# NVIDIA/CUDALibrarySamples

Measured on AMD Instinct MI355X. Metric: contraction GFLOP/s, fp32 einsum abcd,dcbe->ae, higher is better.
Workload: dtype f32

## Files before the change

### cudalibrarysamples_amd/csrc/host/api.cpp

```cpp
#include <algorithm>
#include <cmath>
#include <cstdio>
#include <cstdlib>
#include <cstring>
#include <new>
#include <optional>
#include <sstream>

#include <hip/hip_runtime.h>

#include "internal.hpp"

using namespace ctamd;

static const cutensorComputeDescriptor kCompute[6] = {
    {0, CUTENSOR_COMPUTE_16F}, {1, CUTENSOR_COMPUTE_16BF}, {2, CUTENSOR_COMPUTE_TF32},
    {3, CUTENSOR_COMPUTE_3XTF32}, {4, CUTENSOR_COMPUTE_32F}, {5, CUTENSOR_COMPUTE_64F}};
extern "C" {
const cutensorComputeDescriptor_t CUTENSOR_COMPUTE_DESC_16F    = &kCompute[0];
const cutensorComputeDescriptor_t CUTENSOR_COMPUTE_DESC_16BF   = &kCompute[1];
const cutensorComputeDescriptor_t CUTENSOR_COMPUTE_DESC_TF32   = &kCompute[2];
const cutensorComputeDescriptor_t CUTENSOR_COMPUTE_DESC_3XTF32 = &kCompute[3];
const cutensorComputeDescriptor_t CUTENSOR_COMPUTE_DESC_32F    = &kCompute[4];
const cutensorComputeDescriptor_t CUTENSOR_COMPUTE_DESC_64F    = &kCompute[5];
// ... 1796 lines not shown
        if (h->prof.enabled.load(std::memory_order_relaxed) && hipEventCreate(&e0) == hipSuccess && hipEventCreate(&e1) == hipSuccess)
            (void)hipEventRecord(e0, stream);
    }
    void end() {
        if (!e0 || !e1) return;
        (void)hipEventRecord(e1, stream);
        std::lock_guard<std::mutex> g(handle->prof.mtx);
        handle->prof.events.emplace_back(e0, e1);
    }
};
static bool mode_table_on_device(const cutensorHandle_t handle, cutensorPlan& plan) {
    if (plan.wideDev) return true;
    std::lock_guard<std::mutex> g(handle->mtx);
    if (!plan.wideDev) plan.wideDev = upload_mode_table(plan.wideTab);
    return plan.wideDev != nullptr;
}
static hipError_t launch_mode_table(const cutensorPlan& plan, const GettParams& p, const CallScalars& s, hipStream_t stream) {
    WideParams w = plan.wide;
    w.modes = plan.wideDev.get();
    w.A = p.A; w.B = p.B; w.C = p.C; w.D = p.D;
    w.alpha = p.alpha; w.beta = p.beta; w.alpha64 = s.a; w.beta64 = s.b;
    w.alphaIm = s.aIm; w.betaIm = s.bIm;
    g_launchCounts[1].fetch_add(1, std::memory_order_relaxed);
    return launch_gett_wide(w, (int)plan.dtype, plan.accumulate64, stream);
}
static hipError_t launch_strip_plan(const ContractionChoice& c, const GettKernelInfo& ki, const GettKernelInfo& ks, const GettParams& p, hipStream_t stream) {
    const uint32_t mInt = c.mInt, nInt = c.nInt, Mt = p.gM.total, Nt = p.gN.total, Lt = p.gL.total;
    GettParams q = p;
    q.tilesM = mInt / (uint32_t)ki.bm; q.tilesN = nInt / (uint32_t)ki.bn;
    q.nBlocks = q.tilesM * q.tilesN * Lt;
    const hipError_t err = ki.launch(q, stream);
    GettParams s2 = p;
    s2.mOrg = mInt; s2.nOrg = 0;
    s2.tilesM = (Mt - mInt + (uint32_t)ks.bm - 1u) / (uint32_t)ks.bm; s2.tilesN = (Nt + (uint32_t)ks.bn - 1u) / (uint32_t)ks.bn;
    s2.mOrg2 = 0; s2.nOrg2 = nInt;
    s2.tilesM2 = (mInt + (uint32_t)ks.bm - 1u) / (uint32_t)ks.bm; s2.tilesN2 = (Nt - nInt + (uint32_t)ks.bn - 1u) / (uint32_t)ks.bn;
    if (s2.tilesM * s2.tilesN == 0u) {
        s2.mOrg = s2.mOrg2; s2.nOrg = s2.nOrg2; s2.tilesM = s2.tilesM2; s2.tilesN = s2.tilesN2;
        s2.tilesM2 = s2.tilesN2 = 0;
    }
    s2.nBlocks = (s2.tilesM * s2.tilesN + s2.tilesM2 * s2.tilesN2) * Lt;
    return (err == hipSuccess && s2.nBlocks > 0u) ? ks.launch(s2, stream) : err;
}
static hipError_t launch_tiled(const cutensorHandle_t handle, const cutensorPlan& plan, GettParams& p, const CallScalars& s, void* workspace, hipStream_t stream) {
    const ContractionChoice& c = plan.choice;
    int count = 0;
    const GettKernelInfo* tab = kernel_table(c.family, &count);
    g_launchCounts[2 + c.family].fetch_add(1, std::memory_order_relaxed);
    p.partial = (c.splitK > 1) ? static_cast<float*>(workspace) : nullptr;
    int launchKernel = c.kernel;
    if (c.family == 0) {
        static const int policy = [] { const char* e = CTAMD_HOOK_ENV("CUTENSOR_AMD_PARTIAL_STORE"); return e ? (e[0] == 'p' ? 1 : e[0] == 'n' ? 2 : e[0] == 's' ? 3 : 0) : 0; }();
        p.partialPolicy = policy;
        p.noFlatStart = CTAMD_HOOK_ENV_IS("CUTENSOR_AMD_FLAT_START", '0') ? 1 : 0;
        if (plan.fusedFold) {
            uint32_t slot;
            {
                std::lock_guard<std::mutex> g(handle->mtx);
                slot = handle->syncNext++ % cutensorHandle::kSyncSlots;
            }
            p.sync = handle->syncPool + (size_t)slot * 16;
        }
    } else if (c.family == 1) {
        static const bool persistentForced = CTAMD_HOOK_ENV("CUTENSOR_AMD_H16_WAVES") != nullptr && h16_waves_variant() == H16_W4P;
        if (tab[launchKernel].variant == H16_W4P && s.b != 0.0 && p.cStrideN[0] != 1 && !persistentForced)
            launchKernel = h16_entry(H16_W4X, launchKernel - H16_W4P);
        g_lastH16Kernel.store(launchKernel, std::memory_order_relaxed);
    }
    ProfiledLaunch prof(handle, stream);
    hipError_t err = (c.family == 1 && c.stripKernel >= 0 && c.stripKernel < count) ? launch_strip_plan(c, tab[launchKernel], tab[c.stripKernel], p, stream)
                                                                                    : tab[launchKernel].launch(p, stream);
    prof.end();
    if (err != hipSuccess || c.splitK <= 1 || (c.family == 0 && (plan.fusedFold || handle->skipFold.load(std::memory_order_relaxed)))) return err;
    SplitKReduceParams r = plan.skr;
    r.partial = static_cast<float*>(workspace);
    r.C = p.C; r.D = p.D; r.alpha = p.alpha; r.beta = p.beta;
    r.alpha64 = s.a; r.beta64 = s.b; r.alphaIm = s.aIm; r.betaIm = s.bIm; r.conjC = p.conjC;
    r.noFlatStart = p.noFlatStart;
    return launch_splitk_fold(c.family, tab[c.kernel], r, stream);
}

cutensorStatus_t cutensorContract(const cutensorHandle_t handle, const cutensorPlan_t plan, const void* alpha,
                                  const void* A, const void* B, const void* beta, const void* C, void* D,
                                  void* workspace, uint64_t workspaceSize, cudaStream_t stream) try {
    if (handle == nullptr) return CUTENSOR_STATUS_NOT_INITIALIZED;
    if (plan == nullptr || plan->kind != OpKind::Contraction) return CUTENSOR_STATUS_INVALID_VALUE;
    if (alpha == nullptr || beta == nullptr || A == nullptr || B == nullptr || D == nullptr) return CUTENSOR_STATUS_INVALID_VALUE;
    const CallScalars s{scalar_as_double(alpha, plan->scalarType), scalar_as_double(beta, plan->scalarType), scalar_imag(alpha, plan->scalarType),
                        scalar_imag(beta, plan->scalarType)};
    const bool betaZero = (s.b == 0.0 && s.bIm == 0.0);
    if (!betaZero && C == nullptr) return CUTENSOR_STATUS_INVALID_VALUE;
    if (misaligned(A, plan->alignA) || misaligned(B, plan->alignB) || misaligned(D, plan->alignD) ||
        (!betaZero && misaligned(C, plan->alignC)))
        return CUTENSOR_STATUS_INVALID_VALUE;
    if (plan->requiredWorkspace > 0 && (workspace == nullptr || workspaceSize < plan->requiredWorkspace))
        return CUTENSOR_STATUS_INSUFFICIENT_WORKSPACE;
    switch (plan->planKind) {
        case PlanKind::LoneReduce:
        case PlanKind::Repack: return run_two_step(handle, *plan, alpha, A, B, beta, C, D, workspace, workspaceSize, stream);
        case PlanKind::Peeled: return run_peeled(handle, *plan, alpha, A, B, beta, C, D, workspace, workspaceSize, stream);
        case PlanKind::ModeTable:
            if (!mode_table_on_device(handle, *plan)) return CUTENSOR_STATUS_ALLOC_FAILED;
            break;
        default: break;
    }
    GettParams p = plan->gett;
    p.A = plan->view.swapped ? B : A;
// ... 425 lines not shown
```

### cudalibrarysamples_amd/csrc/kernels/gett_f32_stream.hip

```cpp
#include <hip/hip_runtime.h>
#include <stdint.h>
#include <stdlib.h>

#include <atomic>

#include "params.h"
#include "launch.h"
#include "gett_common.h"

namespace ctamd {

constexpr int kStreamBK = 32;

typedef uint32_t u32x4 __attribute__((ext_vector_type(4)));
#if defined(__HIP_DEVICE_COMPILE__)
typedef __amdgpu_buffer_rsrc_t BufRsrc;
#else
typedef int BufRsrc;
#endif
__device__ __forceinline__ BufRsrc make_rsrc(const float* base, uint32_t records = 0xffffffffu) {
#if defined(__HIP_DEVICE_COMPILE__)
    return __builtin_amdgcn_make_buffer_rsrc(const_cast<float*>(base), 0, (int)records, 0x00020000);
#else
    (void)base; (void)records; return 0;
#endif
}
__device__ __forceinline__ void store_wt_16(f32x4 v, BufRsrc rsrc, uint32_t byteOff) {
#if defined(__HIP_DEVICE_COMPILE__)
    __builtin_amdgcn_raw_buffer_store_b128(__builtin_bit_cast(u32x4, v), rsrc, (int)byteOff, 0,  16);
#else
    (void)v; (void)rsrc; (void)byteOff;
#endif
}
template <int AUX>
__device__ __forceinline__ void store_policy_16(f32x4 v, BufRsrc rsrc, uint32_t byteOff) {
#if defined(__HIP_DEVICE_COMPILE__)
    __builtin_amdgcn_raw_buffer_store_b128(__builtin_bit_cast(u32x4, v), rsrc, (int)byteOff, 0, AUX);
#else
    (void)v; (void)rsrc; (void)byteOff;
#endif
}
template <int AUX = 0>
__device__ __forceinline__ void lds_dma_16(BufRsrc rsrc, uint32_t laneBytes, uint32_t tileBytes, float* dst) {
#if defined(__HIP_DEVICE_COMPILE__)
    __builtin_amdgcn_raw_ptr_buffer_load_lds(rsrc, (__attribute__((address_space(3))) void*)dst, 16, (int)laneBytes, (int)tileBytes, 0, AUX);
#else
    (void)rsrc; (void)laneBytes; (void)tileBytes; (void)dst;
#endif
}

template <int LAY, int ROWS>
struct StreamOperand {
    static_assert(ROWS % 32 == 0, "tile rows must be a multiple of 32");
    static constexpr int PIECES   = ROWS / 8;
    static constexpr int PER_WAVE = PIECES / 4;
    static constexpr int FLOATS   = ROWS * kStreamBK;
    static constexpr int UR       = ROWS / 4;

    uint32_t src[PER_WAVE];

    template <int SLOT_K>
    __device__ __forceinline__ void init(const ModeGroup& gFree, const ModeGroup& gK, uint32_t row0, int wave, int lane) {
        const int64_t strideK0 = gK.stride[SLOT_K][0];
#pragma unroll
        for (int i = 0; i < PER_WAVE; ++i) {
// ... 137 lines not shown
                offB = sgpr((uint32_t)group_offset<1>(gK, k) * 4u);
            }
        }
    }
    __device__ static __forceinline__ uint32_t flat_div(const StreamFlatParams& f, int i, uint32_t n) {
        return __umulhi(n, f.kMagic[i]) >> ((f.kShifts >> (8 * i)) & 0xffu);
    }
    __device__ static __forceinline__ void flat_high(const StreamFlatParams& f, uint32_t hi, uint32_t& a, uint32_t& b) {
        const uint32_t d3 = flat_div(f, 2, hi), d2 = hi - d3 * f.kExt[2];
        a = d2 * f.kStrideA[2] + d3 * f.kStrideA[3];
        b = d2 * f.kStrideB[2] + d3 * f.kStrideB[3];
    }
    __device__ __forceinline__ void init(const StreamFlatParams& f, uint32_t k0) {
        const uint32_t E0 = f.kExt[0];
        n0 = sgpr(E0 / kStreamBK);
        e1 = sgpr(f.kExt[1]);
        const uint32_t q0 = flat_div(f, 0, k0), d0 = k0 - q0 * E0;
        j0 = sgpr(d0 / kStreamBK);
        hi = sgpr((e1 < 2) ? q0 : flat_div(f, 1, q0));
        j1 = sgpr(q0 - hi * e1);
        uint32_t a, b;
        flat_high(f, hi, a, b);
        offA = sgpr(d0 * f.kStrideA[0] + j1 * f.kStrideA[1] + a);
        offB = sgpr(d0 * f.kStrideB[0] + j1 * f.kStrideB[1] + b);
        stepA = sgpr((uint32_t)kStreamBK * f.kStrideA[0]);
        stepB = sgpr((uint32_t)kStreamBK * f.kStrideB[0]);
        wrapA = sgpr(f.kStrideA[1] - (n0 - 1) * stepA);
        wrapB = sgpr(f.kStrideB[1] - (n0 - 1) * stepB);
    }
    __device__ __forceinline__ void advance(const StreamFlatParams& f) {
        const bool c0 = (j0 + 1 == n0);
        j0 = c0 ? 0u : j0 + 1;
        offA += c0 ? wrapA : stepA;
        offB += c0 ? wrapB : stepB;
        j1 += c0 ? 1u : 0u;
        if (j1 == e1) {
            j1 = 0;
            hi += 1;
            if (hi * e1 * f.kExt[0] < f.kTotal) {
                uint32_t a, b;
                flat_high(f, hi, a, b);
                offA = sgpr(a);
                offB = sgpr(b);
            }
        }
    }
};

template <int BM_, int BN_, int LA_, int LB_, int S_, int ABL_ = 0, bool RAG_ = false>
struct StreamCfg {
    static constexpr int BM = BM_, BN = BN_, LA = LA_, LB = LB_, S = S_;
    static constexpr bool RAG = RAG_;
    static constexpr int ABL = ABL_;
    static constexpr bool FLAT = ABL_ == 6 || ABL_ == 7;
    static constexpr bool NT = ABL_ == 5 || ABL_ == 7;
    static constexpr int TM = BM / 32, TN = BN / 32;
};

#define CTAMD_WAIT_VMCNT(n) asm volatile("s_waitcnt vmcnt(%0)" ::"n"(n) : "memory")

template <class Cfg>
__global__ void __launch_bounds__(512, 2) gett_f32_stream_kernel(const GettParams p) {
    constexpr int BM = Cfg::BM, BN = Cfg::BN, BK = kStreamBK, S = Cfg::S;
    constexpr int TM = Cfg::TM, TN = Cfg::TN;
    using OpA = StreamOperand<Cfg::LA, BM>;
    using OpB = StreamOperand<Cfg::LB, BN>;
    constexpr int STAGE = OpA::FLOATS + OpB::FLOATS;
    constexpr int LOADS = OpA::PER_WAVE + OpB::PER_WAVE;
    static_assert(S >= 3 && S <= 6 && S * STAGE * 4 <= 160 * 1024, "LDS ring must fit 160 KiB");
    static_assert(LOADS * (S - 1) <= 63, "vmcnt is a 6-bit counter");
    __shared__ __attribute__((aligned(16))) float lds[S * STAGE];
    prefetch_kernarg<(int)sizeof(GettParams)>();

    const int tid  = threadIdx.x;
    const int lane = tid & 63;
    const int wave8 = __builtin_amdgcn_readfirstlane(tid >> 6);
    const int wave = wave8 & 3;
    const bool loader = wave8 >= 4;
    unsigned long long* tlog = p.timing ? p.timing + (size_t)blockIdx.x * 16 : nullptr;
    auto lane_now = []() -> int {
#if defined(__HIP_DEVICE_COMPILE__)
        return (int)__builtin_amdgcn_mbcnt_hi(~0u, __builtin_amdgcn_mbcnt_lo(~0u, 0u));
#else
        return 0;
#endif
    };
    auto stamp = [&](int slot) {
        if (tlog != nullptr && wave8 == 0 && lane_now() == 0) tlog[slot] = (slot >= 5 && slot != 7) ? wall_clock64() : __builtin_readcyclecounter();
    };
    stamp(0);
    stamp(5);

    uint32_t id = xcd_remap(blockIdx.x, p.nBlocks);
    const uint32_t mt = id % p.tilesM; id /= p.tilesM;
    const uint32_t nt = id % p.tilesN; id /= p.tilesN;
    const uint32_t slice = id % p.splitK;
    const uint32_t l = id / p.splitK;
    const uint32_t m0 = mt * BM, n0 = nt * BN;
    uint32_t kBegin = slice * p.kPerSlice;
    int nTiles;
    if (p.xcdTiles != 0) {
        const uint32_t q = p.splitK >> 3;
        const uint32_t x = slice / q, j = slice - x * q;
        uint32_t first = 0, mine = 0;
#pragma unroll
        for (uint32_t y = 0; y < 8; ++y) {
            const uint32_t ny = (uint32_t)(p.xcdTiles >> (8 * y)) & 0xffu;
            first += (y < x) ? ny * q : 0u;
// ... 185 lines not shown
        for (int i = 0; i < TM; ++i) {
            const uint32_t m = m0 + wm * (BM / 2) + 16 * i + 4 * (laneE >> 4);
            if (m >= Mtot) continue;
            int64_t offDm, offCm;
            group_offset2<1>(p.gM, p.cStrideM, m, offDm, offCm);
#pragma unroll
            for (int j = 0; j < TN; ++j) {
                if (!okN[j]) continue;
                f32x4 val = {alpha * acc[i][j][0], alpha * acc[i][j][1], alpha * acc[i][j][2], alpha * acc[i][j][3]};
                if (beta != 0.f) {
                    const float* c = C + offCm + offCn[j];
                    if (vecC) {
                        const f32x4 cv = *reinterpret_cast<const f32x4*>(c);
                        val[0] += beta * cv[0]; val[1] += beta * cv[1]; val[2] += beta * cv[2]; val[3] += beta * cv[3];
                    } else {
                        int64_t dD, dC1, dC2, dC3;
                        group_offset2<1>(p.gM, p.cStrideM, m + 1, dD, dC1);
                        group_offset2<1>(p.gM, p.cStrideM, m + 2, dD, dC2);
                        group_offset2<1>(p.gM, p.cStrideM, m + 3, dD, dC3);
                        val[0] += beta * c[0];
                        val[1] += beta * C[dC1 + offCn[j]];
                        val[2] += beta * C[dC2 + offCn[j]];
                        val[3] += beta * C[dC3 + offCn[j]];
                    }
                }
                __builtin_nontemporal_store(val, reinterpret_cast<f32x4*>(D + offDm + offDn[j]));
            }
        }
        stamp(4);
        stamp(6);
        return;
    }
#pragma unroll
    for (int i = 0; i < TM; ++i)
#pragma unroll
        for (int r = 0; r < 4; ++r) {
            const uint32_t m = m0 + wm * (BM / 2) + 16 * i + 4 * (laneE >> 4) + r;
            if (m >= Mtot) continue;
            int64_t offDm, offCm;
            group_offset2<1>(p.gM, p.cStrideM, m, offDm, offCm);
#pragma unroll
            for (int j = 0; j < TN; ++j) {
                if (!okN[j]) continue;
                float val = alpha * acc[i][j][r];
                if (beta != 0.f) val += beta * C[offCm + offCn[j]];
                D[offDm + offDn[j]] = val;
            }
        }
    stamp(4);
    stamp(6);
}

template <class Cfg>
__global__ void __launch_bounds__(512, 2) gett_f32_stream_kernel(const StreamFlatParams p) {
    static_assert(Cfg::FLAT && !Cfg::RAG, "the flat entry has no ragged form");
    constexpr int BM = Cfg::BM, BN = Cfg::BN, BK = kStreamBK, S = Cfg::S;
    constexpr int TM = Cfg::TM, TN = Cfg::TN;
    using OpA = StreamOperand<Cfg::LA, BM>;
    using OpB = StreamOperand<Cfg::LB, BN>;
    constexpr int STAGE = OpA::FLOATS + OpB::FLOATS;
    constexpr int LOADS = OpA::PER_WAVE + OpB::PER_WAVE;
    static_assert(S >= 3 && S <= 6 && S * STAGE * 4 <= 160 * 1024, "LDS ring must fit 160 KiB");
    static_assert(LOADS * (S - 1) <= 63, "vmcnt is a 6-bit counter");
    __shared__ __attribute__((aligned(16))) float lds[S * STAGE];

    const int tid  = threadIdx.x;
    const int lane = tid & 63;
    const int wave8 = __builtin_amdgcn_readfirstlane(tid >> 6);
    const int wave = wave8 & 3;
    const bool loader = wave8 >= 4;
    unsigned long long* tlog = p.timing ? p.timing + (size_t)blockIdx.x * 16 : nullptr;
    auto lane_now = []() -> int {
#if defined(__HIP_DEVICE_COMPILE__)
        return (int)__builtin_amdgcn_mbcnt_hi(~0u, __builtin_amdgcn_mbcnt_lo(~0u, 0u));
#else
        return 0;
#endif
    };
    auto stamp = [&](int slot) {
        if (tlog != nullptr && wave8 == 0 && lane_now() == 0) tlog[slot] = (slot >= 5 && slot != 7) ? wall_clock64() : __builtin_readcyclecounter();
    };
    stamp(0);
    stamp(5);

    const uint32_t slice = xcd_remap(blockIdx.x, p.nBlocks);
    const uint32_t kBegin = slice * p.kPerSlice;
    uint32_t kEnd = kBegin + p.kPerSlice;
    if (kEnd > p.kTotal) kEnd = p.kTotal;
    const int nTiles = (int)((kEnd - kBegin) / BK);

    if (loader) {
        const BufRsrc A = make_rsrc(p.A);
        const BufRsrc B = make_rsrc(p.B);
        OpA oa;
        OpB ob;
        oa.init_flat(p.sM, p.Mtot, p.kStrideA[0], wave, lane);
        ob.init_flat(p.sN, p.Ntot, p.kStrideB[0], wave, lane);
        KOdometer odo;
        odo.init(p, kBegin);
        auto issue = [&](int slot) {
            float* stage = lds + slot * STAGE;
            constexpr int AUX = Cfg::NT ? 2 : 0;
            oa.template issue<AUX>(A, odo.offA, stage, wave);
            ob.template issue<AUX>(B, odo.offB, stage + OpA::FLOATS, wave);
            odo.advance(p);
        };
        auto fix_last = [] {};
#include "gett_f32_stream_ring.inc"
    }

#include "gett_f32_stream_kloop.inc"

    const int laneE = lane_now();
    f32x4* P = reinterpret_cast<f32x4*>(p.partial) + ((size_t)slice * 4 + wave) * (size_t)(TM * TN * 64);
    const BufRsrc rP = make_rsrc(reinterpret_cast<const float*>(P));
#pragma unroll
    for (int i = 0; i < TM; ++i)
#pragma unroll
        for (int j = 0; j < TN; ++j) store_wt_16(acc[i][j], rP, (uint32_t)(((i * TN + j) * 64 + laneE) * 16));
    stamp(4);
    stamp(6);
}

__global__ void __launch_bounds__(256) splitk_reduce_frag_kernel(const SplitKReduceParams p) {
    __shared__ f32x4 red[4][8];
    const int q = threadIdx.x & 7, g = threadIdx.x >> 3;
    const uint32_t quadsPerTile = 4u * p.fragTM * p.fragTN * 64u;
    const size_t   tilesTotal = (size_t)p.gL.total * p.tilesN * p.tilesM;
    const size_t   quadsTotal = tilesTotal * quadsPerTile;
    const size_t   e = (size_t)blockIdx.x * 8 + q;
    f32x4 sum = {0.f, 0.f, 0.f, 0.f};
    if (e < quadsTotal) {
        const f32x4* src = reinterpret_cast<const f32x4*>(p.partial) + e;
        for (uint32_t s0 = g; s0 < p.splitK; s0 += 256) {
            f32x4 x[8];
#pragma unroll
            for (int u = 0; u < 8; ++u) {
                const uint32_t sl = s0 + 32u * u;
                x[u] = (sl < p.splitK) ? __builtin_nontemporal_load(src + (size_t)sl * quadsTotal) : f32x4{0.f, 0.f, 0.f, 0.f};
            }
            sum += ((x[0] + x[1]) + (x[2] + x[3])) + ((x[4] + x[5]) + (x[6] + x[7]));
        }
    }
#pragma unroll
    for (int m = 8; m < 64; m <<= 1)
#pragma unroll
        for (int c = 0; c < 4; ++c) sum[c] += __shfl_xor(sum[c], m, 64);
    const int wave = threadIdx.x >> 6;
    if ((threadIdx.x & 63) < 8) red[wave][q] = sum;
    __syncthreads();
    if (threadIdx.x >= 8 || e >= quadsTotal) return;
    sum = (red[0][q] + red[1][q]) + (red[2][q] + red[3][q]);
    size_t rem = e;
    const uint32_t lane = (uint32_t)(rem % 64); rem /= 64;
    const uint32_t j = (uint32_t)(rem % p.fragTN); rem /= p.fragTN;
    const uint32_t i = (uint32_t)(rem % p.fragTM); rem /= p.fragTM;
    const uint32_t w = (uint32_t)(rem % 4); rem /= 4;
    const uint32_t mt = (uint32_t)(rem % p.tilesM); rem /= p.tilesM;
    const uint32_t nt = (uint32_t)(rem % p.tilesN); rem /= p.tilesN;
    const uint32_t l = (uint32_t)rem;
    const uint32_t bm = 32u * p.fragTM, bn = 32u * p.fragTN;
    const uint32_t n = nt * bn + (w >> 1) * (bn / 2) + 16 * j + (lane & 15);
    if (n >= p.gN.total) return;
    int64_t oDl = 0, oCl = 0, oDn, oCn;
    group_offset2<2>(p.gL, p.cStrideL, l, oDl, oCl);
    group_offset2<1>(p.gN, p.cStrideN, n, oDn, oCn);
#pragma unroll
    for (int r = 0; r < 4; ++r) {
        const uint32_t m = mt * bm + (w & 1) * (bm / 2) + 16 * i + 4 * (lane >> 4) + r;
        if (m >= p.gM.total) continue;
        int64_t oDm, oCm;
        group_offset2<1>(p.gM, p.cStrideM, m, oDm, oCm);
        float val = p.alpha * sum[r];
        if (p.beta != 0.f) val += p.beta * static_cast<const float*>(p.C)[oCl + oCm + oCn];
        static_cast<float*>(p.D)[oDl + oDm + oDn] = val;
    }
}

struct FoldFlatParams {
    const float* partial;
    uint32_t     splitK, quadsTotal;
    float*       D;
    const float* C;
    int64_t      sDm, sDn, sCm, sCn;
    float        alpha, beta;
    uint32_t     tilesM, Mtot, Ntot;
    uint32_t     fragTM, fragTN;
};

template <int NT, int FTM, int FTN>
__global__ void __launch_bounds__(NT) splitk_reduce_frag_flat_kernel(const FoldFlatParams p) {
    constexpr int G = NT / 8, U = 256 / G, W = NT / 64;
    __shared__ f32x4 red[W][8];
    const int q = threadIdx.x & 7, g = threadIdx.x >> 3;
    const uint32_t e = blockIdx.x * 8 + q;
    const bool live = e < p.quadsTotal;
    const f32x4* src = reinterpret_cast<const f32x4*>(p.partial) + e;
    auto load = [&](f32x4 (&x)[U], uint32_t s0) {
#pragma unroll
        for (int u = 0; u < U; ++u) {
            const uint32_t sl = s0 + (uint32_t)G * u;
            x[u] = (live && sl < p.splitK) ? __builtin_nontemporal_load(src + (size_t)sl * p.quadsTotal) : f32x4{0.f, 0.f, 0.f, 0.f};
        }
    };
    auto tree = [](f32x4 (&x)[U]) {
#pragma unroll
        for (int st = 1; st < U; st <<= 1)
#pragma unroll
            for (int u = 0; u + st < U; u += 2 * st) x[u] += x[u + st];
    };
    f32x4 x[U];
    load(x, (uint32_t)g);
    const uint32_t fragTM = FTM ? (uint32_t)FTM : p.fragTM, fragTN = FTN ? (uint32_t)FTN : p.fragTN;
    uint32_t rem = e;
    const uint32_t lane = rem % 64; rem /= 64;
    const uint32_t j = rem % fragTN; rem /= fragTN;
    const uint32_t i = rem % fragTM; rem /= fragTM;
    const uint32_t w = rem % 4; rem /= 4;
    const uint32_t mt = (p.tilesM == 1u) ? 0u : rem % p.tilesM;
    const uint32_t nt = (p.tilesM == 1u) ? rem : rem / p.tilesM;
    const uint32_t bm = 32u * fragTM, bn = 32u * fragTN;
    const uint32_t n = nt * bn + (w >> 1) * (bn / 2) + 16 * j + (lane & 15);
    const uint32_t m0 = mt * bm + (w & 1) * (bm / 2) + 16 * i + 4 * (lane >> 4);
    float* d = p.D + (int64_t)m0 * p.sDm + (int64_t)n * p.sDn;
    const float* c = p.C + (int64_t)m0 * p.sCm + (int64_t)n * p.sCn;
    tree(x);
    f32x4 sum = {0.f, 0.f, 0.f, 0.f};
    sum += x[0];
    for (uint32_t s0 = g + 256u; s0 < p.splitK; s0 += 256) {
        load(x, s0);
        tree(x);
        sum += x[0];
    }
#pragma unroll
    for (int m = 8; m < 64; m <<= 1)
#pragma unroll
        for (int cc = 0; cc < 4; ++cc) sum[cc] += __shfl_xor(sum[cc], m, 64);
    const int wave = threadIdx.x >> 6;
    if ((threadIdx.x & 63) < 8) red[wave][q] = sum;
    __syncthreads();
    if (threadIdx.x >= 8 || !live || n >= p.Ntot) return;
    sum = red[0][q];
#pragma unroll
    for (int ww = 1; ww < W; ++ww) sum += red[ww][q];
    if (p.beta == 0.f) {
#pragma unroll
        for (int r = 0; r < 4; ++r)
            if (m0 + r < p.Mtot) d[r * p.sDm] = p.alpha * sum[r];
        return;
    }
#pragma unroll
    for (int r = 0; r < 4; ++r) {
        if (m0 + r >= p.Mtot) continue;
        float val = p.alpha * sum[r];
        val += p.beta * c[r * p.sCm];
        d[r * p.sDm] = val;
    }
}

hipError_t launch_splitk_reduce_frag(const SplitKReduceParams& p, hipStream_t stream) {
    const size_t quads = (size_t)p.gL.total * p.tilesN * p.tilesM * 4u * p.fragTM * p.fragTN * 64u;
    const size_t blocks = (quads + 7) / 8;
    if (blocks == 0) return hipSuccess;
    if (p.gL.total == 1 && p.gM.n <= 1 && p.gN.n <= 1 && quads < (1ull << 31)) {
        FoldFlatParams f;
        f.partial = p.partial;
        f.C = static_cast<const float*>(p.C);
        f.D = static_cast<float*>(p.D);
        f.sDm = p.gM.stride[1][0]; f.sDn = p.gN.stride[1][0];
        f.sCm = p.cStrideM[0];     f.sCn = p.cStrideN[0];
        f.alpha = p.alpha; f.beta = p.beta;
        f.splitK = p.splitK; f.quadsTotal = (uint32_t)quads;
        f.fragTM = p.fragTM; f.fragTN = p.fragTN; f.tilesM = p.tilesM;
        f.Mtot = p.gM.total; f.Ntot = p.gN.total;
        const dim3 grid((unsigned)blocks), block(256);
        const uint32_t frag = (p.noFlatStart == 0 && p.fragTM == p.fragTN) ? p.fragTM : 0u;
        if (frag == 2u) hipLaunchKernelGGL((splitk_reduce_frag_flat_kernel<256, 2, 2>), grid, block, 0, stream, f);
        else if (frag == 3u) hipLaunchKernelGGL((splitk_reduce_frag_flat_kernel<256, 3, 3>), grid, block, 0, stream, f);
        else if (frag == 4u) hipLaunchKernelGGL((splitk_reduce_frag_flat_kernel<256, 4, 4>), grid, block, 0, stream, f);
        else hipLaunchKernelGGL((splitk_reduce_frag_flat_kernel<256, 0, 0>), grid, block, 0, stream, f);
        return hipGetLastError();
    }
    hipLaunchKernelGGL(splitk_reduce_frag_kernel, dim3((unsigned)blocks), dim3(256), 0, stream, p);
    return hipGetLastError();
}

std::atomic<uint64_t> g_flatStartLaunches{0};

static bool flat_start_params(const GettParams& p, StreamFlatParams& f) {
    if (p.noFlatStart != 0 || p.partial == nullptr || p.sync != nullptr || p.xcdTiles != 0 || p.partialPolicy != 0) return false;
    if (p.gL.total != 1 || p.gM.n > 1 || p.gN.n > 1 || p.tilesM * p.tilesN != 1 || p.nBlocks != p.splitK) return false;
    if (p.gK.total % (uint32_t)kStreamBK != 0u || p.gK.div[0].d % (uint32_t)kStreamBK != 0u || (p.ragged & 1u) != 0u) return false;
    f.A = static_cast<const float*>(p.A);
    f.B = static_cast<const float*>(p.B);
    f.partial = p.partial;
    f.timing = p.timing;
    f.sM = (uint32_t)p.gM.stride[0][0] * 4u; f.sN = (uint32_t)p.gN.stride[0][0] * 4u;
    f.Mtot = p.gM.total; f.Ntot = p.gN.total;
    f.splitK = p.splitK; f.kPerSlice = p.kPerSlice; f.nBlocks = p.nBlocks;
    f.kTotal = p.gK.total;
    f.kShifts = 0;
    for (int i = 0; i < kMaxGroupModes; ++i) {
        f.kExt[i] = p.gK.div[i].d;
        f.kStrideA[i] = (uint32_t)p.gK.stride[0][i] * 4u;
        f.kStrideB[i] = (uint32_t)p.gK.stride[1][i] * 4u;
        if (i < kMaxGroupModes - 1) {
            f.kMagic[i] = p.gK.div[i].magic;
            f.kShifts |= (p.gK.div[i].shift & 0xffu) << (8 * i);
        }
    }
    return true;
}

template <class Cfg>
static hipError_t launch_stream(const GettParams& p, hipStream_t stream) {
    if constexpr (Cfg::ABL == 0) {
        if (p.gK.total % (uint32_t)kStreamBK != 0u || (p.ragged & 1u) != 0u) {
            using R = StreamCfg<Cfg::BM, Cfg::BN, Cfg::LA, Cfg::LB, 4, 0, true>;
            hipLaunchKernelGGL(gett_f32_stream_kernel<R>, dim3(p.nBlocks), dim3(512), 0, stream, p);
            return hipGetLastError();
        }
    }
    if constexpr (Cfg::BM == 96 && Cfg::BN == 96 && Cfg::S == 3 && (Cfg::ABL == 0 || Cfg::ABL == 5)) {
        StreamFlatParams f;
        if (flat_start_params(p, f)) {
            using F = StreamCfg<96, 96, Cfg::LA, Cfg::LB, 3, Cfg::ABL == 0 ? 6 : 7>;
            hipLaunchKernelGGL(gett_f32_stream_kernel<F>, dim3(p.nBlocks), dim3(512), 0, stream, f);
            g_flatStartLaunches.fetch_add(1, std::memory_order_relaxed);
            return hipGetLastError();
        }
    }
    hipLaunchKernelGGL(gett_f32_stream_kernel<Cfg>, dim3(p.nBlocks), dim3(512), 0, stream, p);
    return hipGetLastError();
}

#define CTAMD_STREAM_KERNELS(XS)        \
    XS(96, 96, LAY_K, LAY_F, 4)         \
    XS(96, 96, LAY_K, LAY_F, 6)         \
    XS(96, 96, LAY_K, LAY_F, 3)         \
    XS(96, 96, LAY_F, LAY_F, 4)         \
    XS(96, 96, LAY_F, LAY_K, 4)         \
    XS(96, 96, LAY_K, LAY_K, 4)         \
    XS(128, 128, LAY_F, LAY_F, 4)       \
    XS(128, 128, LAY_K, LAY_F, 4)       \
    XS(128, 128, LAY_F, LAY_K, 4)       \
    XS(128, 128, LAY_K, LAY_K, 4)       \
    XS(64, 64, LAY_F, LAY_F, 4)         \
    XS(64, 64, LAY_K, LAY_F, 4)         \
    XS(64, 64, LAY_F, LAY_K, 4)         \
    XS(64, 64, LAY_K, LAY_K, 4)         \
    XS(96, 96, LAY_F, LAY_F, 3)         \
    XS(96, 96, LAY_F, LAY_K, 3)         \
    XS(96, 96, LAY_K, LAY_K, 3)         \
    XS(128, 128, LAY_F, LAY_F, 3)       \
    XS(128, 128, LAY_K, LAY_F, 3)

#define CTAMD_STREAM_ENTRY(bm, bn, la, lb, s) \
    {bm, bn, kStreamBK, 2, 2, 1, la, lb, 512, s, 1, 0, &launch_stream<StreamCfg<bm, bn, la, lb, s>>, 1, 0, 0, 0, "gett_f32_stream_kernel"},

#define CTAMD_STREAM_ABL(bm, bn, la, lb, s, abl) \
    {bm, bn, kStreamBK, 2, 2, 1, la, lb, 512, s, 1, abl, &launch_stream<StreamCfg<bm, bn, la, lb, s, abl>>, 1, 0, 0, 0, "gett_f32_stream_kernel"},

#define CTAMD_STREAM_NT(bm, bn, la, lb, s) \
    {bm, bn, kStreamBK, 2, 2, 1, la, lb, 512, s, 1, 0, &launch_stream<StreamCfg<bm, bn, la, lb, s, 5>>, 1, 1, 0, 0, "gett_f32_stream_kernel"},

static const GettKernelInfo g_stream_table[] = {
    CTAMD_STREAM_KERNELS(CTAMD_STREAM_ENTRY)
    CTAMD_STREAM_ABL(96, 96, LAY_K, LAY_F, 4, 1)
    CTAMD_STREAM_ABL(96, 96, LAY_K, LAY_F, 4, 2)
    CTAMD_STREAM_ABL(96, 96, LAY_K, LAY_F, 4, 3)
    CTAMD_STREAM_ABL(96, 96, LAY_K, LAY_F, 4, 4)
    CTAMD_STREAM_NT(96, 96, LAY_K, LAY_F, 3) CTAMD_STREAM_NT(96, 96, LAY_F, LAY_F, 3)
    CTAMD_STREAM_NT(96, 96, LAY_F, LAY_K, 3) CTAMD_STREAM_NT(96, 96, LAY_K, LAY_K, 3)};

const GettKernelInfo* gett_f32_stream_kernels(int* count) {
    *count = (int)(sizeof(g_stream_table) / sizeof(g_stream_table[0]));
    return g_stream_table;
}

}
```

### cudalibrarysamples_amd/csrc/kernels/gett_f32_stream_kloop.inc

```
    __builtin_amdgcn_s_setprio(2);
    const int wm = wave & 1, wn = wave >> 1;
    f32x4 acc[TM][TN];
#pragma unroll
    for (int i = 0; i < TM; ++i)
#pragma unroll
        for (int j = 0; j < TN; ++j) acc[i][j] = f32x4{0.f, 0.f, 0.f, 0.f};

    int baseA[TM], baseB[TN];
#pragma unroll
    for (int i = 0; i < TM; ++i) baseA[i] = OpA::frag_base(wm * (BM / 2) + 16 * i, lane);
#pragma unroll
    for (int j = 0; j < TN; ++j) baseB[j] = OpB::frag_base(wn * (BN / 2) + 16 * j, lane);

    f32x4 a0[TM], b0[TN], a1[TM], b1[TN];
    auto load0 = [&](const float* st) {
#pragma unroll
        for (int i = 0; i < TM; ++i) a0[i] = OpA::template fragment<0>(st, baseA[i]);
#pragma unroll
        for (int j = 0; j < TN; ++j) b0[j] = OpB::template fragment<0>(st + OpA::FLOATS, baseB[j]);
    };
    auto load1 = [&](const float* st) {
#pragma unroll
        for (int i = 0; i < TM; ++i) a1[i] = OpA::template fragment<1>(st, baseA[i]);
#pragma unroll
// ... 10 lines not shown
    constexpr int NMFMA = 4 * TM * TN;
    constexpr int SPLIT = NMFMA / 3;
#define CTAMD_INTERLEAVE_DS(n)                                         \
    _Pragma("unroll") for (int z = 0; z < (n); ++z) {                  \
        __builtin_amdgcn_sched_group_barrier(0x008, 1, 0);             \
        __builtin_amdgcn_sched_group_barrier(0x100, 1, 0);             \
    }

    __builtin_amdgcn_s_barrier();
    __builtin_amdgcn_sched_barrier(0);
    load0(lds);
    stamp(1);
    unsigned long long waitC = 0;

#define CTAMD_TILE_BODY(U, LASTTILE) CTAMD_TILE_BODY_AT(lds + (U) * STAGE, lds + (((U) + 1) % S) * STAGE, LASTTILE)
#define CTAMD_TILE_BODY_AT(CUR, NXT, LASTTILE) CTAMD_TILE_BODY_AT2(CUR, NXT, LASTTILE, load0, load1)
#define CTAMD_TILE_BODY_AT2(CUR, NXT, LASTTILE, load0, load1)                                              \
    {                                                                                                      \
        const float* cur = (CUR);                                                                          \
        const float* nxt = (NXT);                                                                          \
        load1(cur);                                                                                        \
        CTAMD_MFMA_RANGE(a0, b0, 0, NMFMA)                                                                 \
        CTAMD_INTERLEAVE_DS(TM + 4 * TN)                                                                   \
        __builtin_amdgcn_sched_barrier(0);                                                                 \
        CTAMD_MFMA_RANGE(a1, b1, 0, SPLIT)                                                                 \
        __builtin_amdgcn_sched_barrier(0);                                                                 \
        if constexpr (!(LASTTILE)) {                                                                       \
            asm volatile("s_waitcnt lgkmcnt(0)" ::: "memory");  \
            unsigned long long cb0 = 0;                                                                    \
            if constexpr (Cfg::ABL == 3) cb0 = __builtin_readcyclecounter();                               \
            __builtin_amdgcn_s_barrier();                                                                  \
            if constexpr (Cfg::ABL == 3) waitC += __builtin_readcyclecounter() - cb0;                      \
            __builtin_amdgcn_sched_barrier(0);                                                             \
            load0(nxt);                                                                                    \
            CTAMD_MFMA_RANGE(a1, b1, SPLIT, NMFMA)                                                         \
            CTAMD_INTERLEAVE_DS(TM + 4 * TN)                                                               \
        } else {                                                                                           \
            CTAMD_MFMA_RANGE(a1, b1, SPLIT, NMFMA)                                                         \
        }                                                                                                  \
        __builtin_amdgcn_sched_barrier(0);                                                                 \
    }
#define CTAMD_BODY_MID(U) CTAMD_TILE_BODY(U, false)
#define CTAMD_FOR_SLOTS(M)                                                     \
    { M(0) M(1) M(2)                                                           \
      if constexpr (S > 3) { M(3) } if constexpr (S > 4) { M(4) }              \
      if constexpr (S > 5) { M(5) } }
    int t = 0;
    for (; t + S < nTiles; t += S) CTAMD_FOR_SLOTS(CTAMD_BODY_MID)
    stamp(2);
    const int r = nTiles - t;
#define CTAMD_BODY_END(U) CTAMD_TILE_BODY(U, (U) == S - 1)
    if (r == S) {
        CTAMD_FOR_SLOTS(CTAMD_BODY_END)
    } else {
        auto opaque = [](int v) { asm volatile("" : "+v"(v)); return v; };
        auto load0t = [&](const float* st) {
#pragma unroll
            for (int i = 0; i < TM; ++i) a0[i] = OpA::template fragment<0>(st, opaque(baseA[i]));
#pragma unroll
            for (int j = 0; j < TN; ++j) b0[j] = OpB::template fragment<0>(st + OpA::FLOATS, opaque(baseB[j]));
        };
        auto load1t = [&](const float* st) {
#pragma unroll
            for (int i = 0; i < TM; ++i) a1[i] = OpA::template fragment<1>(st, opaque(baseA[i]));
#pragma unroll
            for (int j = 0; j < TN; ++j) b1[j] = OpB::template fragment<1>(st + OpA::FLOATS, opaque(baseB[j]));
        };
        int u = 0;
#pragma unroll 1
        for (; u + 1 < r; ++u) CTAMD_TILE_BODY_AT2(lds + u * STAGE, lds + (u + 1) * STAGE, false, load0t, load1t)
        CTAMD_TILE_BODY_AT2(lds + u * STAGE, lds, true, load0t, load1t)
    }
    stamp(3);
    if constexpr (Cfg::ABL == 3) {
        if (tlog != nullptr && wave8 == 0 && lane_now() == 0) tlog[8] = waitC;
    }
```

### cudalibrarysamples_amd/csrc/kernels/params.h

```cpp
#pragma once
#include <stdint.h>

namespace ctamd {

constexpr int kMaxGroupModes = 4;

struct FastDiv {
    uint32_t d;
    uint32_t magic;
    uint32_t shift;
};

struct ModeGroup {
    int32_t  n;
    uint32_t total;
    FastDiv  div[kMaxGroupModes];
    int64_t  stride[3][kMaxGroupModes];
};

struct GettParams {
    const void* A;
    const void* B;
    const void* C;
    void*       D;
    float*      partial;
    unsigned long long* timing;
    uint32_t*   sync;
    unsigned long long xcdTiles;
    ModeGroup   gM, gN, gK, gL;
    float       alpha, beta;
    double      alpha64, beta64;
    uint32_t    tilesM, tilesN;
    uint32_t    splitK;
    uint32_t    kPerSlice;
    uint32_t    nBlocks;
    int64_t     cStrideM[kMaxGroupModes];
    int64_t     cStrideN[kMaxGroupModes];
    int64_t     cStrideL[kMaxGroupModes];
    double      alphaIm, betaIm;
    int32_t     conjA, conjB, conjC;
    int32_t     partialPolicy;
    unsigned long long endA, endB;
    uint32_t    ragged;
    uint32_t    mOrg, nOrg;
    uint32_t    tilesM2, tilesN2, mOrg2, nOrg2;
    int32_t     noFlatStart;
};

struct StreamFlatParams {
    const float* A;
    const float* B;
    float*       partial;
    unsigned long long* timing;
    uint32_t     sM, sN;
    uint32_t     Mtot, Ntot;
    uint32_t     splitK, kPerSlice, nBlocks;
    uint32_t     kTotal;
    uint32_t     kExt[kMaxGroupModes];
    uint32_t     kMagic[kMaxGroupModes - 1];
    uint32_t     kShifts;
    uint32_t     kStrideA[kMaxGroupModes], kStrideB[kMaxGroupModes];
};
static_assert(sizeof(StreamFlatParams) == 128, "the flat entry's arguments are two 64-byte lines");

struct WideMode {
    FastDiv div;
    int64_t sA, sB, sC, sD;
};
struct WideParams {
    const void* A;
    const void* B;
    const void* C;
    void*       D;
    const WideMode* modes;
    uint32_t    nOut, nK;
    uint64_t    outTotal;
    uint32_t    kTotal;
    float       alpha, beta;
    double      alpha64, beta64;
    double      alphaIm, betaIm;
    int32_t     conjA, conjB, conjC;
};

struct SplitKReduceParams {
    const float* partial;
    const void*  C;
    void*        D;
    ModeGroup    gM, gN, gL;
    int64_t      cStrideM[kMaxGroupModes];
    int64_t      cStrideN[kMaxGroupModes];
    int64_t      cStrideL[kMaxGroupModes];
    float        alpha, beta;
    uint32_t     splitK;
    uint32_t     tilesM, tilesN;
    uint32_t     fragTM, fragTN;
    int32_t      outType;
    double       alpha64, beta64, alphaIm, betaIm;
    int32_t      conjC;
    int32_t      noFlatStart;
};

struct Ew2DParams {
    const void* A;
    const void* C;
    void*       D;
    uint32_t    E0, E1;
    int64_t     sA0, sA1, sD0, sD1, sC0, sC1;
    uint32_t    tiles0, tiles1;
    uint32_t    tile0;
    uint32_t    tile1;
    uint32_t    order;
    uint32_t    idsPerXcd;
    FastDiv     divRest;
    FastDiv     divTiles0, divTiles1;
    ModeGroup   rest;
    uint32_t    nBlocks;
// ... 41 lines not shown
```

Measured before the change: 119,300.

## Pass flat split-K kernel arguments as scalars and straighten the ring tail

Adds argument-list entry points for the flat split-K GETT kernel and its fold kernel, so the values needed first arrive as direct kernel arguments and the rest sit in a single 64-byte tail struct. The K-odometer parameters are made to depend on the issued loads through an empty asm, which defers their scalar loads until after the first global loads are in flight. The partial ring drain for the 3-stage flat kernel is unrolled into straight-line code instead of the generic opaque path. The aim is to cut kernel start-up latency on small, launch-bound contractions, at the cost of extra kernel variants and packing Mtot and Ntot into 16 bits each.

```diff
diff --git a/cudalibrarysamples_amd/csrc/host/api.cpp b/cudalibrarysamples_amd/csrc/host/api.cpp
--- a/cudalibrarysamples_amd/csrc/host/api.cpp
+++ b/cudalibrarysamples_amd/csrc/host/api.cpp
@@ -1872,7 +1872,11 @@
     if (c.family == 0) {
         static const int policy = [] { const char* e = CTAMD_HOOK_ENV("CUTENSOR_AMD_PARTIAL_STORE"); return e ? (e[0] == 'p' ? 1 : e[0] == 'n' ? 2 : e[0] == 's' ? 3 : 0) : 0; }();
         p.partialPolicy = policy;
-        p.noFlatStart = CTAMD_HOOK_ENV_IS("CUTENSOR_AMD_FLAT_START", '0') ? 1 : 0;
+        {
+            const char* e = CTAMD_HOOK_ENV("CUTENSOR_AMD_FLAT_START");
+            p.noFlatStart = (e == nullptr) ? FLAT_START_ARGS : e[0] == '0' ? FLAT_START_GENERAL : e[0] == '2' ? FLAT_START_STRUCT
+                            : e[0] == '3' ? FLAT_START_ARGS_FOLD : e[0] == '4' ? FLAT_START_ARGS_GETT : FLAT_START_ARGS;
+        }
         if (plan.fusedFold) {
             uint32_t slot;
             {
diff --git a/cudalibrarysamples_amd/csrc/kernels/gett_f32_stream.hip b/cudalibrarysamples_amd/csrc/kernels/gett_f32_stream.hip
--- a/cudalibrarysamples_amd/csrc/kernels/gett_f32_stream.hip
+++ b/cudalibrarysamples_amd/csrc/kernels/gett_f32_stream.hip
@@ -11,6 +11,10 @@
 namespace ctamd {
 
 constexpr int kStreamBK = 32;
+
+#ifndef CTAMD_FLAT_STRAIGHT_TAIL
+#define CTAMD_FLAT_STRAIGHT_TAIL 1
+#endif
 
 typedef uint32_t u32x4 __attribute__((ext_vector_type(4)));
 #if defined(__HIP_DEVICE_COMPILE__)
@@ -254,8 +258,8 @@
     static constexpr int BM = BM_, BN = BN_, LA = LA_, LB = LB_, S = S_;
     static constexpr bool RAG = RAG_;
     static constexpr int ABL = ABL_;
-    static constexpr bool FLAT = ABL_ == 6 || ABL_ == 7;
-    static constexpr bool NT = ABL_ == 5 || ABL_ == 7;
+    static constexpr bool FLAT = ABL_ >= 6 && ABL_ <= 9;
+    static constexpr bool NT = ABL_ == 5 || ABL_ == 7 || ABL_ == 9;
     static constexpr int TM = BM / 32, TN = BN / 32;
 };
 
@@ -547,7 +551,13 @@
 }
 
 template <class Cfg>
-__global__ void __launch_bounds__(512, 2) gett_f32_stream_kernel(const StreamFlatParams p) {
+struct StreamFlatRing {
+    static constexpr int STAGE = StreamOperand<Cfg::LA, Cfg::BM>::FLOATS + StreamOperand<Cfg::LB, Cfg::BN>::FLOATS;
+    static constexpr int FLOATS = Cfg::S * STAGE;
+};
+
+template <class Cfg>
+__device__ __forceinline__ void gett_f32_stream_flat_body(const StreamFlatParams& p, float* lds) {
     static_assert(Cfg::FLAT && !Cfg::RAG, "the flat entry has no ragged form");
     constexpr int BM = Cfg::BM, BN = Cfg::BN, BK = kStreamBK, S = Cfg::S;
     constexpr int TM = Cfg::TM, TN = Cfg::TN;
@@ -557,7 +567,6 @@
     constexpr int LOADS = OpA::PER_WAVE + OpB::PER_WAVE;
     static_assert(S >= 3 && S <= 6 && S * STAGE * 4 <= 160 * 1024, "LDS ring must fit 160 KiB");
     static_assert(LOADS * (S - 1) <= 63, "vmcnt is a 6-bit counter");
-    __shared__ __attribute__((aligned(16))) float lds[S * STAGE];
 
     const int tid  = threadIdx.x;
     const int lane = tid & 63;
@@ -591,14 +600,30 @@
         OpB ob;
         oa.init_flat(p.sM, p.Mtot, p.kStrideA[0], wave, lane);
         ob.init_flat(p.sN, p.Ntot, p.kStrideB[0], wave, lane);
+        StreamFlatParams f = p;
+        if constexpr (Cfg::ABL >= 8) {
+            uint32_t done = 0;
+#pragma unroll
+            for (int i = 0; i < OpA::PER_WAVE; ++i) done |= oa.src[i];
+#pragma unroll
+            for (int i = 0; i < OpB::PER_WAVE; ++i) done |= ob.src[i];
+            auto behind = [&](uint32_t& v) { asm volatile("" : "+s"(v) : "v"(done)); };
+#pragma unroll
+            for (int i = 0; i < kMaxGroupModes; ++i) {
+                behind(f.kExt[i]);
+                if (i > 0) { behind(f.kStrideA[i]); behind(f.kStrideB[i]); }
+                if (i < kMaxGroupModes - 1) behind(f.kMagic[i]);
+            }
+            behind(f.kShifts);
+        }
         KOdometer odo;
-        odo.init(p, kBegin);
+        odo.init(f, kBegin);
         auto issue = [&](int slot) {
             float* stage = lds + slot * STAGE;
             constexpr int AUX = Cfg::NT ? 2 : 0;
             oa.template issue<AUX>(A, odo.offA, stage, wave);
             ob.template issue<AUX>(B, odo.offB, stage + OpA::FLOATS, wave);
-            odo.advance(p);
+            odo.advance(f);
         };
         auto fix_last = [] {};
 #include "gett_f32_stream_ring.inc"
@@ -615,6 +640,32 @@
         for (int j = 0; j < TN; ++j) store_wt_16(acc[i][j], rP, (uint32_t)(((i * TN + j) * 64 + laneE) * 16));
     stamp(4);
     stamp(6);
+}
+
+template <class Cfg>
+__global__ void __launch_bounds__(512, 2) gett_f32_stream_kernel(const StreamFlatParams p) {
+    __shared__ __attribute__((aligned(16))) float lds[StreamFlatRing<Cfg>::FLOATS];
+    gett_f32_stream_flat_body<Cfg>(p, lds);
+}
+
+template <class Cfg>
+__global__ void __launch_bounds__(512, 2) gett_f32_stream_kernel(const float* A, const float* B, unsigned long long* timing, uint32_t nBlocks,
+                                                                 uint32_t kPerSlice, uint32_t kTotal, uint32_t sM, uint32_t sN, uint32_t mnTot,
+                                                                 uint32_t kStrideA0, uint32_t kStrideB0, const StreamFlatTail t) {
+    __shared__ __attribute__((aligned(16))) float lds[StreamFlatRing<Cfg>::FLOATS];
+    StreamFlatParams p;
+    p.A = A; p.B = B; p.partial = t.partial; p.timing = timing;
+    p.sM = sM; p.sN = sN; p.Mtot = mnTot & 0xffffu; p.Ntot = mnTot >> 16;
+    p.splitK = nBlocks; p.kPerSlice = kPerSlice; p.nBlocks = nBlocks; p.kTotal = kTotal;
+#pragma unroll
+    for (int i = 0; i < kMaxGroupModes; ++i) {
+        p.kExt[i] = t.kExt[i];
+        p.kStrideA[i] = (i == 0) ? kStrideA0 : t.kStrideA[i > 0 ? i - 1 : 0];
+        p.kStrideB[i] = (i == 0) ? kStrideB0 : t.kStrideB[i > 0 ? i - 1 : 0];
+        if (i < kMaxGroupModes - 1) p.kMagic[i] = t.kMagic[i];
+    }
+    p.kShifts = t.kShifts;
+    gett_f32_stream_flat_body<Cfg>(p, lds);
 }
 
 __global__ void __launch_bounds__(256) splitk_reduce_frag_kernel(const SplitKReduceParams p) {
@@ -684,9 +735,8 @@
 };
 
 template <int NT, int FTM, int FTN>
-__global__ void __launch_bounds__(NT) splitk_reduce_frag_flat_kernel(const FoldFlatParams p) {
+__device__ __forceinline__ void splitk_fold_frag_flat_body(const FoldFlatParams& p, f32x4 (*red)[8]) {
     constexpr int G = NT / 8, U = 256 / G, W = NT / 64;
-    __shared__ f32x4 red[W][8];
     const int q = threadIdx.x & 7, g = threadIdx.x >> 3;
     const uint32_t e = blockIdx.x * 8 + q;
     const bool live = e < p.quadsTotal;
@@ -753,6 +803,27 @@
     }
 }
 
+template <int NT, int FTM, int FTN>
+__global__ void __launch_bounds__(NT) splitk_reduce_frag_flat_kernel(const FoldFlatParams p) {
+    __shared__ f32x4 red[NT / 64][8];
+    splitk_fold_frag_flat_body<NT, FTM, FTN>(p, red);
+}
+
+template <int NT, int FTM, int FTN>
+__global__ void __launch_bounds__(NT) splitk_fold_frag_args_kernel(const float* partial, uint32_t splitK, uint32_t quadsTotal, float* D, int64_t sDm,
+                                                                   int64_t sDn, uint32_t tilesM, uint32_t Mtot, uint32_t Ntot, float alpha, float beta,
+                                                                   const float* C, int64_t sCm, int64_t sCn, uint32_t fragTM, uint32_t fragTN) {
+    __shared__ f32x4 red[NT / 64][8];
+    FoldFlatParams p;
+    p.partial = partial; p.splitK = splitK; p.quadsTotal = quadsTotal;
+    p.D = D; p.C = C;
+    p.sDm = sDm; p.sDn = sDn; p.sCm = sCm; p.sCn = sCn;
+    p.alpha = alpha; p.beta = beta;
+    p.tilesM = tilesM; p.Mtot = Mtot; p.Ntot = Ntot;
+    p.fragTM = fragTM; p.fragTN = fragTN;
+    splitk_fold_frag_flat_body<NT, FTM, FTN>(p, red);
+}
+
 hipError_t launch_splitk_reduce_frag(const SplitKReduceParams& p, hipStream_t stream) {
     const size_t quads = (size_t)p.gL.total * p.tilesN * p.tilesM * 4u * p.fragTM * p.fragTN * 64u;
     const size_t blocks = (quads + 7) / 8;
@@ -769,7 +840,17 @@
         f.fragTM = p.fragTM; f.fragTN = p.fragTN; f.tilesM = p.tilesM;
         f.Mtot = p.gM.total; f.Ntot = p.gN.total;
         const dim3 grid((unsigned)blocks), block(256);
-        const uint32_t frag = (p.noFlatStart == 0 && p.fragTM == p.fragTN) ? p.fragTM : 0u;
+        const uint32_t frag = (p.noFlatStart != FLAT_START_GENERAL && p.fragTM == p.fragTN) ? p.fragTM : 0u;
+        if (p.noFlatStart == FLAT_START_ARGS || p.noFlatStart == FLAT_START_ARGS_FOLD) {
+#define CTAMD_FOLD_ARGS(FT) hipLaunchKernelGGL((splitk_fold_frag_args_kernel<256, FT, FT>), grid, block, 0, stream, f.partial, f.splitK, f.quadsTotal, f.D, \
+                                               f.sDm, f.sDn, f.tilesM, f.Mtot, f.Ntot, f.alpha, f.beta, f.C, f.sCm, f.sCn, f.fragTM, f.fragTN)
+            if (frag == 2u) CTAMD_FOLD_ARGS(2);
+            else if (frag == 3u) CTAMD_FOLD_ARGS(3);
+            else if (frag == 4u) CTAMD_FOLD_ARGS(4);
+            else CTAMD_FOLD_ARGS(0);
+#undef CTAMD_FOLD_ARGS
+            return hipGetLastError();
+        }
         if (frag == 2u) hipLaunchKernelGGL((splitk_reduce_frag_flat_kernel<256, 2, 2>), grid, block, 0, stream, f);
         else if (frag == 3u) hipLaunchKernelGGL((splitk_reduce_frag_flat_kernel<256, 3, 3>), grid, block, 0, stream, f);
         else if (frag == 4u) hipLaunchKernelGGL((splitk_reduce_frag_flat_kernel<256, 4, 4>), grid, block, 0, stream, f);
@@ -783,7 +864,7 @@
 std::atomic<uint64_t> g_flatStartLaunches{0};
 
 static bool flat_start_params(const GettParams& p, StreamFlatParams& f) {
-    if (p.noFlatStart != 0 || p.partial == nullptr || p.sync != nullptr || p.xcdTiles != 0 || p.partialPolicy != 0) return false;
+    if (p.noFlatStart == FLAT_START_GENERAL || p.partial == nullptr || p.sync != nullptr || p.xcdTiles != 0 || p.partialPolicy != 0) return false;
     if (p.gL.total != 1 || p.gM.n > 1 || p.gN.n > 1 || p.tilesM * p.tilesN != 1 || p.nBlocks != p.splitK) return false;
     if (p.gK.total % (uint32_t)kStreamBK != 0u || p.gK.div[0].d % (uint32_t)kStreamBK != 0u || (p.ragged & 1u) != 0u) return false;
     f.A = static_cast<const float*>(p.A);
@@ -819,9 +900,25 @@
     if constexpr (Cfg::BM == 96 && Cfg::BN == 96 && Cfg::S == 3 && (Cfg::ABL == 0 || Cfg::ABL == 5)) {
         StreamFlatParams f;
         if (flat_start_params(p, f)) {
+            g_flatStartLaunches.fetch_add(1, std::memory_order_relaxed);
+            if (p.noFlatStart == FLAT_START_ARGS || p.noFlatStart == FLAT_START_ARGS_GETT) {
+                using F = StreamCfg<96, 96, Cfg::LA, Cfg::LB, 3, Cfg::ABL == 0 ? 8 : 9>;
+                StreamFlatTail t;
+                t.partial = f.partial;
+                t.kShifts = f.kShifts;
+                for (int i = 0; i < kMaxGroupModes; ++i) {
+                    t.kExt[i] = f.kExt[i];
+                    if (i < kMaxGroupModes - 1) { t.kMagic[i] = f.kMagic[i]; t.kStrideA[i] = f.kStrideA[i + 1]; t.kStrideB[i] = f.kStrideB[i + 1]; }
+                }
+                void (*kernel)(const float*, const float*, unsigned long long*, uint32_t, uint32_t, uint32_t, uint32_t, uint32_t, uint32_t, uint32_t, uint32_t,
+                               const StreamFlatTail) = gett_f32_stream_kernel<F>;
+                hipLaunchKernelGGL(kernel, dim3(p.nBlocks), dim3(512), 0, stream, f.A, f.B, f.timing, f.nBlocks, f.kPerSlice, f.kTotal, f.sM, f.sN,
+                                   f.Mtot | (f.Ntot << 16), f.kStrideA[0], f.kStrideB[0], t);
+                return hipGetLastError();
+            }
             using F = StreamCfg<96, 96, Cfg::LA, Cfg::LB, 3, Cfg::ABL == 0 ? 6 : 7>;
-            hipLaunchKernelGGL(gett_f32_stream_kernel<F>, dim3(p.nBlocks), dim3(512), 0, stream, f);
-            g_flatStartLaunches.fetch_add(1, std::memory_order_relaxed);
+            void (*kernel)(const StreamFlatParams) = gett_f32_stream_kernel<F>;
+            hipLaunchKernelGGL(kernel, dim3(p.nBlocks), dim3(512), 0, stream, f);
             return hipGetLastError();
         }
     }
diff --git a/cudalibrarysamples_amd/csrc/kernels/gett_f32_stream_kloop.inc b/cudalibrarysamples_amd/csrc/kernels/gett_f32_stream_kloop.inc
--- a/cudalibrarysamples_amd/csrc/kernels/gett_f32_stream_kloop.inc
+++ b/cudalibrarysamples_amd/csrc/kernels/gett_f32_stream_kloop.inc
@@ -86,6 +86,14 @@
 #define CTAMD_BODY_END(U) CTAMD_TILE_BODY(U, (U) == S - 1)
     if (r == S) {
         CTAMD_FOR_SLOTS(CTAMD_BODY_END)
+    } else if constexpr (Cfg::FLAT && CTAMD_FLAT_STRAIGHT_TAIL) {
+        static_assert(S == 3, "the flat entries run the 3-deep ring");
+        if (r == 2) {
+            CTAMD_TILE_BODY(0, false)
+            CTAMD_TILE_BODY(1, true)
+        } else {
+            CTAMD_TILE_BODY(0, true)
+        }
     } else {
         auto opaque = [](int v) { asm volatile("" : "+v"(v)); return v; };
         auto load0t = [&](const float* st) {
diff --git a/cudalibrarysamples_amd/csrc/kernels/params.h b/cudalibrarysamples_amd/csrc/kernels/params.h
--- a/cudalibrarysamples_amd/csrc/kernels/params.h
+++ b/cudalibrarysamples_amd/csrc/kernels/params.h
@@ -47,6 +47,14 @@
     int32_t     noFlatStart;
 };
 
+enum FlatStart : int32_t {
+    FLAT_START_ARGS = 0,
+    FLAT_START_GENERAL = 1,
+    FLAT_START_STRUCT = 2,
+    FLAT_START_ARGS_FOLD = 3,
+    FLAT_START_ARGS_GETT = 4
+};
+
 struct StreamFlatParams {
     const float* A;
     const float* B;
@@ -62,6 +70,15 @@
     uint32_t     kStrideA[kMaxGroupModes], kStrideB[kMaxGroupModes];
 };
 static_assert(sizeof(StreamFlatParams) == 128, "the flat entry's arguments are two 64-byte lines");
+
+struct StreamFlatTail {
+    uint32_t     kExt[kMaxGroupModes];
+    uint32_t     kMagic[kMaxGroupModes - 1];
+    uint32_t     kShifts;
+    uint32_t     kStrideA[kMaxGroupModes - 1], kStrideB[kMaxGroupModes - 1];
+    float*       partial;
+};
+static_assert(sizeof(StreamFlatTail) == 64, "one line, one round of scalar loads");
 
 struct WideMode {
     FastDiv div;
```

After: 120,900, median of 6. 1.3% higher.
